# JuliaCrypto/ToyFHE.jl

Measured on AMD Instinct MI355X. Metric: ciphertext-mul/s (BFV ct*ct + relinearize, N=2^14, L=8 RNS), higher is better.
Workload: dtype u64; 1 GPU; BFV N=2^14, L=8 RNS limbs (50-bit primes), extension basis 17 limbs, t=65537, ciphertext-mul + relinearize (RNS-digit keyswitch), bit-exact; batch_per_gpu=1024, global_batch=1024

## Files before the change

toyfhe.jl_amd/csrc/kernels.h:

```cpp
#pragma once
#include <hip/hip_runtime.h>
#include <type_traits>
#include "bfv_core.h"
#include "bfv_fast.h"
#include "lazy_sum.h"
#include "ntt_core.h"

typedef u64 u64x2_t __attribute__((ext_vector_type(2)));

#ifndef TFHE_NTT_WAVES
#define TFHE_NTT_WAVES 2
#endif

__device__ __forceinline__ u32 fresh_tid() {
    u32 t = threadIdx.x;
    asm volatile("" : "+v"(t));
    return t;
}

struct limb_sel_t {
    int n;
    int idx[TFHE_MAX_LIMBS];
};


template <class A, int LOGB, int LOGT, int S0>
__device__ __forceinline__ void fwd_schedule(u64* lds, const u64* gsrc, u64* gdst, const typename A::ctx& C, u32 tid,
                                             u32 pre, int x, u32 sbrev, const lift_t* lift) {
    constexpr int K = pass_k_fwd(LOGB, LOGT, S0);
    constexpr bool LAST = (S0 + K == LOGB);
    ntt_fwd_pass<A, LOGB, LOGT, S0, K, S0 == 0, LAST>(lds, gsrc, gdst, C, tid, pre, x, sbrev, lift);
    if constexpr (!LAST) {
        __syncthreads();
        fwd_schedule<A, LOGB, LOGT, S0 + K>(lds, gsrc, gdst, C, tid, pre, x, sbrev, lift);
    }
}
template <class A, int LOGB, int LOGT, int SEND, bool SCALE = true, class AO = A>
__device__ __forceinline__ void inv_schedule_ptw(u64* lds, const u64* gsrc, u64* gdst, const typename A::ctx& C, u32 tid,
                                                 u32 pre, const u64* addend, const typename A::tw* tw_cur, u64* keep = nullptr) {
    constexpr int K = pass_k_inv(LOGB, LOGT, SEND);
    constexpr int S0 = SEND - K;
    constexpr bool FROM_GLOBAL = (SEND == LOGB), TO_GLOBAL = (S0 == 0);
    typedef pgeom<LOGB, LOGT, S0, K> G;
    u64 raw[G::E];
    typename A::elem v[G::E];
    inv_load_data<LOGB, LOGT, S0, K, FROM_GLOBAL>(raw, lds, gsrc, tid, 0, 0u);
    inv_compute<A, LOGB, LOGT, S0, K, FROM_GLOBAL, SCALE, (TO_GLOBAL || FROM_GLOBAL) ? 0 : K>(v, raw, tw_cur, C, tid, pre);
    if constexpr (!TO_GLOBAL) {
        constexpr int K2 = pass_k_inv(LOGB, LOGT, S0);
        typedef pgeom<LOGB, LOGT, S0 - K2, K2> G2;
        typename A::tw tw_next[G2::SETS * G2::NTW];
        if constexpr (S0 - K2 != 0) inv_load_tw<A, LOGB, LOGT, S0 - K2, K2, false>(tw_next, C, tid, pre);
        inv_store<A, LOGB, LOGT, S0, K, FROM_GLOBAL, SCALE>(v, lds, gdst, C, tid, nullptr);
        __syncthreads();
        inv_schedule_ptw<A, LOGB, LOGT, S0, SCALE, AO>(lds, gsrc, gdst, C, tid, pre, addend, tw_next, keep);
    } else {
        inv_store<AO, LOGB, LOGT, S0, K, FROM_GLOBAL, SCALE>(v, lds, gdst, C, tid, addend, keep);
    }
}

template <class A, int LOGB, int LOGT, int SEND, bool SCALE>
__device__ __forceinline__ void inv_schedule(u64* lds, const u64* gsrc, u64* gdst, const typename A::ctx& C, u32 tid,
                                             u32 pre, int x, u32 sbrev, const u64* addend) {
    constexpr int K = pass_k_inv(LOGB, LOGT, SEND);
    constexpr int S0 = SEND - K;
    ntt_inv_pass<A, LOGB, LOGT, S0, K, SEND == LOGB, S0 == 0, SCALE>(lds, gsrc, gdst, C, tid, pre, x, sbrev, addend);
    if constexpr (S0 != 0) {
        __syncthreads();
        inv_schedule<A, LOGB, LOGT, S0, SCALE>(lds, gsrc, gdst, C, tid, pre, x, sbrev, addend);
    }
}

__device__ __forceinline__ u32 xcd_walk_item(u32 it, u32 b, u32 grid, int x, u32 nitems) {
    const u32 nsb = 1u << x;
    if (x == 0 || (grid % (8u * nsb)) != 0u) {
        const u32 item = it * grid + b;
        return item < nitems ? item : ~0u;
    }
    const u32 xcd = b & 7u, slot = b >> 3, groups = (grid >> 3) >> x;
    const u32 row = it * (8u * groups) + xcd * groups + (slot >> x);
    const u32 item = (row << x) | (slot & (nsb - 1u));
    return item < nitems ? item : ~0u;
}
__device__ __forceinline__ u32 xcd_limb_niter(u32 grid, u32 nitems) {
    if (grid & 7u) return (nitems + grid - 1) / grid;
    const u32 per = (nitems + 7u) >> 3, nslots = grid >> 3;
    return (per + nslots - 1) / nslots;
}
__device__ __forceinline__ u32 xcd_limb_walk(u32 it, u32 wg, u32 grid, u32 nb, u32 nitems) {
    if (grid & 7u) {
        const u32 item = it * grid + wg;
        return item < nitems ? item : ~0u;
    }
    const u32 per = (nitems + 7u) >> 3, nslots = grid >> 3, xcd = wg & 7u, slot = wg >> 3;
    const u32 k = it * nslots + slot, idx = xcd * per + k;
    if (k >= per || idx >= nitems) return ~0u;
    const u32 B = nitems / nb, j = idx / B, b = idx - j * B;
    return b * nb + j;
}
__device__ __forceinline__ u32 dense_mask(u32 limbs, u32 mask) { return (limbs & 1u) ? 0u : mask; }
__device__ __forceinline__ u32 dense_count(u32 nitems, int x, u32 limbs, u32 mask) {
    return mask ? ((((nitems >> x) / limbs) * (u32)__popc(mask)) << x) : nitems;
}
__device__ __forceinline__ u32 dense_item(u32 d, int x, u32 limbs, u32 mask) {
    if (!mask || d == ~0u) return d;
    const u32 nact = (u32)__popc(mask), sb = d & ((1u << x) - 1u), pld = d >> x, g = pld / nact, a = pld % nact;
    u32 m = mask;
    for (u32 i = 0; i < a; i++) m &= m - 1u;
    return ((g * limbs + (u32)__ffs((int)m) - 1u) << x) | sb;
}
template <class A, int LOGB, int LOGT, int IOMODE>
__global__ __launch_bounds__(1 << LOGT, TFHE_NTT_WAVES) void k_ntt_fwd_block(const u64* __restrict__ src, u64* __restrict__ dst,
                                                              const ntt_limb_t* __restrict__ LT, limb_sel_t sel, int x,
                                                              u32 nitems, ntt_io_t io) {
    extern __shared__ __attribute__((aligned(16))) u64 lds[];
    const size_t ntot = (size_t)1 << (LOGB + x);
    const u32 dmask = dense_mask((u32)sel.n, io.limb_mask), dn = dense_count(nitems, x, (u32)sel.n, dmask), niter = (dn + gridDim.x - 1) / gridDim.x;
    bool first = true;
    for (u32 it = 0; it < niter; it++) {
        const u32 item = dense_item(xcd_walk_item(it, blockIdx.x, gridDim.x, x, dn), x, (u32)sel.n, dmask);
        if (item == ~0u) continue;
        const u32 sb = item & ((1u << x) - 1), pl = item >> x;
        u32 srow = pl, drow = pl, j = pl % (u32)sel.n;
        lift_t lf;
        const lift_t* lift = nullptr;
        if constexpr (IOMODE == 1) {
            const u32 per_ct = io.level * io.nw, b = pl / per_ct, rem = pl % per_ct, i = rem / io.nw;
            j = rem % io.nw;
            srow = (b * io.polys + io.polys - 1) * io.level + i;
            const ntt_limb_t& Li = LT[sel.idx[i]];
            const ntt_limb_t& Lj = LT[sel.idx[j]];
            lf.qi = Li.q; lf.half = Li.q >> 1; lf.qj = Lj.q; lf.bj = Lj.br;
            if (io.lift_unsigned) lf.qi = lf.half = ~0ull;
            lift_wide_consts<A>(lf);
            lift = &lf;
        }
        if (io.limb_mask && !((io.limb_mask >> j) & 1u)) continue;
        const typename A::ctx C = A::make(LT[sel.idx[j]]);
        if (!first) __syncthreads();
        first = false;
// ... 1201 lines not shown
        u32 mk0[DCH][2], mk1[DCH][2], md0[DCH][2], md1[DCH][2];
#pragma unroll
        for (int ii = 0; ii < DCH; ii++) {
            const int i = i0 + ii < A.level ? i0 + ii : A.level - 1;
            const u64x2_t a = *(const u64x2_t*)(evk + (((size_t)i * 2 + 0) * Lk + A.w.idx[j]) * n + k);
            const u64x2_t d = *(const u64x2_t*)(evk + (((size_t)i * 2 + 1) * Lk + A.w.idx[j]) * n + k);
#pragma unroll
            for (int v = 0; v < 2; v++) {
                mk0[ii][v] = (u32)a[v] & 0x3ffffffu; mk1[ii][v] = (u32)(a[v] >> 26);
                md0[ii][v] = (u32)d[v] & 0x3ffffffu; md1[ii][v] = (u32)(d[v] >> 26);
            }
        }
        for (u32 b = b_lo; b < b_hi; b++) {
            constexpr bool pairs = EPI;
            u64x2_t *s1p, *s2p;
            if (EPI) {
                s1p = (u64x2_t*)(S + epi_pair(b, j, k, (u32)A.nw, n));
                s2p = s1p + 1;
            } else {
                s1p = (u64x2_t*)(S + (((size_t)b * 2 + 0) * A.nw + j) * n + k);
                s2p = (u64x2_t*)(S + (((size_t)b * 2 + 1) * A.nw + j) * n + k);
            }
            u64x2_t p1 = {0, 0}, p2 = {0, 0};
            if (i0) {
                p1 = *s1p; p2 = *s2p;
                if (pairs) { const u64x2_t a = p1, c = p2; p1.x = a.x; p1.y = c.x; p2.x = a.y; p2.y = c.y; }
            }
            acc52 s1[2] = {{p1[0], 0, 0}, {p1[1], 0, 0}}, s2[2] = {{p2[0], 0, 0}, {p2[1], 0, 0}};
            u64x2_t dv[DCH];
#pragma unroll
            for (int ii = 0; ii < DCH; ii++)
                if (i0 + ii < A.level) dv[ii] = *(const u64x2_t*)(dig + (((size_t)b * A.level + i0 + ii) * A.nw + j) * n + k);
#pragma unroll
            for (int ii = 0; ii < DCH; ii++) {
                if (i0 + ii < A.level) {
#pragma unroll
                    for (int v = 0; v < 2; v++) {
                        const u32 d0 = (u32)dv[ii][v] & 0x3ffffffu, d1 = (u32)(dv[ii][v] >> 26);
                        acc52_mac(s1[v], d0, d1, md0[ii][v], md1[ii][v]);
                        acc52_mac(s2[v], d0, d1, mk0[ii][v], mk1[ii][v]);
                    }
                }
            }
            u64x2_t r1, r2;
#pragma unroll
            for (int v = 0; v < 2; v++) {
                u64 lo, hi;
                acc52_fold(s1[v], lo, hi);
                r1[v] = barrett_reduce128(lo, hi, br);
                acc52_fold(s2[v], lo, hi);
                r2[v] = barrett_reduce128(lo, hi, br);
            }
            if constexpr (EPI) {
                if (i0 + DCH >= A.level && j < (u32)K.epi_level) {
                    const u64x2_t x = *(const u64x2_t*)(K.epi_x + (((size_t)b * 2) * K.epi_level + j) * n + k);
#pragma unroll
                    for (int v = 0; v < 2; v++) {
                        r1[v] = addmod(shoup_full(r1[v], A.pinv[j], br.q), x[v], br.q);
                        r2[v] = shoup_full(r2[v], A.pinv[j], br.q);
                    }
                }
            }
            if (pairs) {
                u64x2_t a, c;
                a.x = r1[0]; a.y = r2[0]; c.x = r1[1]; c.y = r2[1];
                *s1p = a;
                *s2p = c;
            } else {
                *s1p = r1;
                *s2p = r2;
            }
        }
    }
}

template <class A, int LOGB, int LOGT, bool PRELIFT = false>
__device__ __forceinline__ void fused_fwd_to_regs(u64* lds, const u64* grow, const typename A::ctx& C, bool& first,
                                                  typename A::elem* v, const lift_t* lift = nullptr) {
    constexpr int K1 = pass_k_fwd(LOGB, LOGT, 0), K2 = pass_k_fwd(LOGB, LOGT, K1), K3 = LOGB - K1 - K2;
    constexpr int E = 1 << (LOGB - LOGT);
    const u32 tid = fresh_tid();
    {
        u64 raw[E];
        fwd_load_data<LOGB, LOGT, 0, K1, true, false>(raw, lds, grow, tid);
        if (!first) __syncthreads();
        first = false;
        if constexpr (PRELIFT) {
#pragma unroll
            for (int i = 0; i < E; i++) pin_vgpr(raw[i]);
            TFHE_SCHED_FENCE();
            fwd_compute<A, LOGB, LOGT, 0, K1, false, false, 0>(v, raw, nullptr, C, tid, 1u);
        } else {
            fwd_compute<A, LOGB, LOGT, 0, K1, true, false, 0>(v, raw, nullptr, C, tid, 1u, lift);
        }
        fwd_store<A, LOGB, LOGT, 0, K1, false>(v, lds, nullptr, C, tid, 0, 0u);
    }
    __syncthreads();
    ntt_fwd_pass<A, LOGB, LOGT, K1, K2, false, false>(lds, nullptr, nullptr, C, tid, 1u, 0, 0u);
    __syncthreads();
    {
        u64 r3[E];
        fwd_load_data<LOGB, LOGT, K1 + K2, K3, false, true>(r3, lds, nullptr, tid);
        fwd_compute<A, LOGB, LOGT, K1 + K2, K3, false, true, 0>(v, r3, nullptr, C, tid, 1u);
    }
}
template <class A, int LOGB, int LOGT, bool SCALE = true, class AO = A>
__device__ __forceinline__ void fused_inv_from_regs(u64* lds, typename A::elem* v, u64* gdst, const typename A::ctx& C, const u64* addend,
                                                    u64* keep = nullptr, u32 pre = 1u) {
    constexpr int KI1 = pass_k_inv(LOGB, LOGT, LOGB);
    constexpr int E = 1 << (LOGB - LOGT);
    const u32 tid = fresh_tid();
    __syncthreads();
    constexpr int S1 = LOGB - KI1, K2 = pass_k_inv(LOGB, LOGT, S1);
    typedef pgeom<LOGB, LOGT, S1 - K2, K2> G2;
    typename A::tw tw_next[G2::SETS * G2::NTW];
    {
#pragma unroll
        for (int e = 0; e < E; e++) v[e] = fp_reduce(v[e], C.p, C.pinv);
        inv_compute<A, LOGB, LOGT, S1, KI1, true, SCALE, 0, -1, no_hook, true>(v, nullptr, nullptr, C, tid, pre);
        if constexpr (S1 - K2 != 0) inv_load_tw<A, LOGB, LOGT, S1 - K2, K2, false>(tw_next, C, tid, pre);
        inv_store<A, LOGB, LOGT, S1, KI1, true, SCALE>(v, lds, nullptr, C, tid);
    }
    __syncthreads();
    inv_schedule_ptw<A, LOGB, LOGT, S1, SCALE, AO>(lds, nullptr, gdst, C, tid, pre, addend, tw_next, keep);
}

template <class A, int LOGB, int LOGT>
__global__ __launch_bounds__(1 << LOGT) void k_ntt_inv_quad2(const u64* __restrict__ src, u64* __restrict__ dst,
                                                              const ntt_limb_t* __restrict__ LT, limb_sel_t sel, u32 nitems, u32 limb_mask) {
    extern __shared__ __attribute__((aligned(16))) u64 lds[];
    constexpr int x = 2;
    constexpr int K1 = pass_k_inv(LOGB, LOGT, LOGB), S1 = LOGB - K1;
    typedef pgeom<LOGB, LOGT, S1, K1> G1;
    constexpr int E = G1::E;
    constexpr int K2 = pass_k_inv(LOGB, LOGT, S1), KL = S1 - K2;
    static_assert(KL >= 1 && pass_k_inv(LOGB, LOGT, KL) == KL, "three-pass schedule expected");
    typedef pgeom<LOGB, LOGT, 0, KL> GL;
    static_assert(GL::SETS == 1 && GL::LO == LOGT, "last pass: element r of a thread is word tid + (r << LOGT)");
    static_assert(G1::SETS << (LOGT + K1) == 1 << LOGB, "first pass: register position e <-> point tid + (e << LOGT)");
    const size_t ntot = (size_t)1 << (LOGB + x);
    const u32 dmask = dense_mask((u32)sel.n, limb_mask), dn = dense_count(nitems, 1, (u32)sel.n, dmask), niter = (dn + gridDim.x - 1) / gridDim.x;
    bool first = true;
    for (u32 it = 0; it < niter; it++) {
        const u32 item = dense_item(xcd_walk_item(it, blockIdx.x, gridDim.x, x - 1, dn), 1, (u32)sel.n, dmask);
        if (item == ~0u) continue;
        const u32 ph = item & 1u, pl = item >> 1, j = pl % (u32)sel.n;
        if (limb_mask && !((limb_mask >> j) & 1u)) continue;
        const ntt_limb_t& L = LT[sel.idx[j]];
        typename A::ctx C = A::make(L);
        C.Winvb = L.i2_winvb;
        const u64* s = src + pl * ntot;
        u64* d = dst + pl * ntot + 2u * ph;
        typename A::elem w[2][E];
        {
            const u32 tid = fresh_tid();
            typedef __attribute__((address_space(1))) const double* gptr_t;
            const gptr_t t0 = (gptr_t)L.i2_t0;
            double ta = ph ? t0[(1u << LOGT) + tid] : 1.0;
            double tb = t0[(ph ? (2u << LOGT) : 0u) + tid];
            const ftw_t ga{ph ? L.i2_g[1] : 1.0}, gb{ph ? L.i2_g[2] : L.i2_g[0]}, iinv{L.i2_iinv};
            const double sgn = ph ? -1.0 : 1.0;
            pin_vgpr(ta);
            pin_vgpr(tb);
            if (!first) __syncthreads();
            dma_stream_load<LOGB, LOGT, 4, 2>(lds, s, tid, [&](int e, const u64* q) {
                const int idx = (e % G1::SETS) * G1::R + (int)brev_bits((u32)(e / G1::SETS), K1);
                const double a0 = fp_from_u64(q[0]), a1 = fp_from_u64(q[1]), a2 = fp_from_u64(q[2]), a3 = fp_from_u64(q[3]);
                asm volatile("" : "+v"(ta), "+v"(tb) : "v"(a0));
                const double slo = fp_fma(sgn, a1 + a3, a0 + a2);
                const double t = fp_mulmod_c(a1 - a3, iinv, C.p, C.pinv);
                const double shi = fp_fma(sgn, t, a0 - a2);
                w[0][idx] = fp_mulmod_c(slo, ftw_t{ta}, C.p, C.pinv);
                w[1][idx] = fp_mulmod_c(shi, ftw_t{tb}, C.p, C.pinv);
                ta = fp_mulmod_c(ta, ga, C.p, C.pinv);
                tb = fp_mulmod_c(tb, gb, C.p, C.pinv);
            });
            first = false;
            TFHE_SCHED_FENCE();
        }
        u64 held[E];
#pragma unroll
        for (int half = 0; half < 2; half++) {
            const u32 tid = fresh_tid();
            TFHE_SCHED_FENCE();
            __syncthreads();
            {
                typename A::elem* v = w[half];
#pragma unroll
                for (int e = 0; e < E; e++) v[e] = fp_reduce(v[e], C.p, C.pinv);
                inv_compute<A, LOGB, LOGT, S1, K1, true, true, 0, -1, no_hook, true>(v, nullptr, nullptr, C, tid, 1u);
                inv_store<A, LOGB, LOGT, S1, K1, true, true>(v, lds, nullptr, C, tid);
            }
            __syncthreads();
            ntt_inv_pass<A, LOGB, LOGT, KL, K2, false, false, true>(lds, nullptr, nullptr, C, tid, 1u, 0, 0u);
            __syncthreads();
            {
                u64 r3[E];
                typename A::elem v[E];
                inv_load_data<LOGB, LOGT, 0, KL, false>(r3, lds, nullptr, tid, 0, 0u);
                inv_compute<A, LOGB, LOGT, 0, KL, false, true, 0>(v, r3, nullptr, C, tid, 1u);
                if (half == 0) {
#pragma unroll
                    for (int r = 0; r < E; r++) held[r] = A::out_inv_scaled(v[r], C);
                } else {
#pragma unroll
                    for (int r = 0; r < E; r++) {
                        u64x2_t ww;
// ... 26 lines not shown
        d[pair ? pos * 2 : pos] = b;
    }
}
template <int LOGB, int LOGT>
constexpr size_t fused_lds_bytes() {
    return (size_t)lds_words<LOGB, LOGT>() * 8;
}
template <class A, int LOGB, int LOGT, bool PRELIFT = false, int SPMODE = 0>
__global__ __launch_bounds__(1 << LOGT) void k_ks_fused(const u64* __restrict__ evd, const u64* __restrict__ ct,
                                                         u64* __restrict__ out, const ntt_limb_t* __restrict__ LT,
                                                         ks_arg_t KA, int Lk, u32 nitems, const u64* __restrict__ tsp = nullptr,
                                                         const u64* __restrict__ zero_row = nullptr) {
    extern __shared__ __attribute__((aligned(16))) u64 lds[];
    constexpr int K1 = pass_k_fwd(LOGB, LOGT, 0), K2 = pass_k_fwd(LOGB, LOGT, K1), K3 = LOGB - K1 - K2;
    static_assert(K3 >= 1 && pass_k_fwd(LOGB, LOGT, K1 + K2) == K3, "three-pass forward schedule expected");
    constexpr int KI1 = pass_k_inv(LOGB, LOGT, LOGB);
    static_assert(KI1 == K3, "forward last pass and inverse first pass must share the register map");
    typedef pgeom<LOGB, LOGT, 0, K1> G1;
    typedef pgeom<LOGB, LOGT, K1 + K2, K3> G3;
    constexpr int E = G3::E;
    const u32 level = (u32)KA.level, polys = (u32)KA.polys, nw = (u32)KA.nw;
    const u32 add_s = polys == 3 ? 2u : 1u;
    bool first = true;
    const u32 niter = (nitems + gridDim.x - 1) / gridDim.x;
    for (u32 it = 0; it < niter; it++) {
        const u32 nper = SPMODE == 1 ? 1u : (SPMODE >= 2 ? level : nw);
        const u32 item = it * gridDim.x + blockIdx.x;
        if (item >= nitems) break;
        const u32 b = item / nper, j = SPMODE == 1 ? level : item % nper;
        const ntt_limb_t& Lj = LT[KA.w.idx[j]];
        typename A::ctx C = A::make(Lj);
        lift_t lf;
        lf.qj = Lj.q;
        lf.bj = Lj.br;
        typename A::elem acc[2][E];
#pragma unroll
        for (int e = 0; e < E; e++) acc[0][e] = acc[1][e] = 0;
        for (u32 i = 0; i < level; i++) {
            const u32 tid = fresh_tid();
            lf.qi = LT[KA.w.idx[i]].q;
            lf.half = lf.qi >> 1;
            const u64* grow = ct + ((size_t)((b * polys + polys - 1) * level + i) << LOGB);
            typename A::elem v[E];
            fused_fwd_to_regs<A, LOGB, LOGT, PRELIFT>(lds, grow, C, first, v, &lf);
            const u64x2_t* e_pair = (const u64x2_t*)(evd + ((((size_t)i * nw + j) << LOGB) << 1));
#pragma unroll
            for (int u = 0; u < G3::SETS; u++) {
                u32 c0, hi, base;
                G3::template coords<true>(tid, u, c0, hi, base);
#pragma unroll
                for (int r = 0; r < G3::R; r++) {
                    const u32 nat = (brev_bits((u32)r, K3) << (LOGB - K3)) + c0;
                    const int e = u * G3::R + r;
                    const u64x2_t kw = e_pair[nat];
                    const typename A::tw k1{A::from_lds(kw.y)}, k0{A::from_lds(kw.x)};
                    const double y = A::pre_product(v[e], C);
                    acc[0][e] += fp_mulmod_c(y, k1, C.p, C.pinv);
                    acc[1][e] += fp_mulmod_c(y, k0, C.p, C.pinv);
                }
            }
            if ((i & 7u) == 7u && i + 1 < level) {
#pragma unroll
                for (int e = 0; e < E; e++) {
                    acc[0][e] = fp_reduce(acc[0][e], C.p, C.pinv);
                    acc[1][e] = fp_reduce(acc[1][e], C.p, C.pinv);
                }
            }
        }
#pragma unroll
        for (int sidx = 0; sidx < 2; sidx++) {
            if constexpr (SPMODE >= 2) {
                C.md_pinv = (double)KA.pinv[j].w;
                C.md_c = (u32)sidx < add_s ? ct + ((size_t)((b * polys + sidx) * level + j) << LOGB) : zero_row;
                C.md_g = KA.rot_g;
                u64* gdst = out + ((size_t)((b * 2 + sidx) * level + j) << LOGB);
                typedef typename std::conditional<SPMODE == 3, ArithFpMDR, ArithFpMD>::type AOUT;
                fused_inv_from_regs<A, LOGB, LOGT, false, AOUT>(lds, acc[sidx], gdst, C, tsp + ((size_t)(b * 2 + sidx) << LOGB));
            } else if constexpr (SPMODE == 1) {
                u64* gdst = out + ((size_t)(b * 2 + sidx) << LOGB);
                fused_inv_from_regs<A, LOGB, LOGT, false>(lds, acc[sidx], gdst, C, nullptr);
            } else {
                const u64* addend = (!KA.special && (u32)sidx < add_s) ? ct + ((size_t)((b * polys + sidx) * level + j) << LOGB) : nullptr;
                u64* gdst = out + ((size_t)((b * 2 + sidx) * nw + j) << LOGB);
                fused_inv_from_regs<A, LOGB, LOGT, false>(lds, acc[sidx], gdst, C, addend);
            }
        }
    }
}

template <class A, int LOGB, int LOGT, int X>
__global__ __launch_bounds__(1 << LOGT) void k_ks_fused_sub(const u64* __restrict__ evd, const u64* __restrict__ ct,
                                                             u64* __restrict__ T, const ntt_limb_t* __restrict__ LT,
                                                             ks_arg_t KA, int Lk, u32 nitems) {
    extern __shared__ __attribute__((aligned(16))) u64 lds[];
    constexpr int K1 = pass_k_fwd(LOGB, LOGT, 0), K2 = pass_k_fwd(LOGB, LOGT, K1), K3 = LOGB - K1 - K2;
    static_assert(K3 >= 1 && pass_k_fwd(LOGB, LOGT, K1 + K2) == K3, "three-pass forward schedule expected");
    constexpr int KI1 = pass_k_inv(LOGB, LOGT, LOGB), S1 = LOGB - KI1;
    static_assert(KI1 == K3, "forward last pass and inverse first pass must share the register map");
    typedef pgeom<LOGB, LOGT, K1 + K2, K3> G3;
    constexpr int E = G3::E;
    const u32 level = (u32)KA.level, polys = (u32)KA.polys, nw = (u32)KA.nw;
    const u32 niter = (nitems + gridDim.x - 1) / gridDim.x;
    bool first = true;
    for (u32 it = 0; it < niter; it++) {
        const u32 item = xcd_walk_item(it, blockIdx.x, gridDim.x, X, nitems);
        if (item == ~0u) continue;
        const u32 sb = item & ((1u << X) - 1u), pl = item >> X, b = pl / nw, j = pl % nw, pre = (1u << X) + sb;
        const ntt_limb_t& Lj = LT[KA.w.idx[j]];
        const typename A::ctx C = A::make(Lj);
        lift_t lf;
        lf.qj = Lj.q;
        lf.bj = Lj.br;
        const typename A::tw w1 = A::ld_fwd(C, 1u), w2 = A::ld_fwd(C, 2u + (sb >> 1));
        const double sgn_h = (sb >> (X - 1)) ? -1.0 : 1.0, sgn_q = (sb & 1u) ? -1.0 : 1.0;
        typename A::elem acc[2][E];
#pragma unroll
        for (int e = 0; e < E; e++) acc[0][e] = acc[1][e] = 0;
        for (u32 i = 0; i < level; i++) {
            const u32 tid = fresh_tid();
            lf.qi = LT[KA.w.idx[i]].q;
            lf.half = lf.qi >> 1;
            const u64* grow = ct + ((size_t)((b * polys + polys - 1) * level + i) << (LOGB + X));
            typename A::elem v[E];
            {
                u64 op[E];
                constexpr int PC = 4 * X, PE = E / PC;
                if constexpr (X == 2) {
                    if (!first) __syncthreads();
                    dma_stream_load<LOGB, LOGT, 1 << X, 2>(lds, grow, tid, [&](int e, const u64* q) {
                        double xin[1 << X];
#pragma unroll
                        for (int m = 0; m < (1 << X); m++) xin[m] = A::from_global_lift(q[m], C, lf, true);
                        double z;
                        if constexpr (X == 1) {
                            z = fp_fma(sgn_h, fp_mulmod_c(xin[1], w1, C.p, C.pinv), xin[0]);
                        } else {
                            const double ya = fp_fma(sgn_h, fp_mulmod_c(xin[2], w1, C.p, C.pinv), xin[0]);
                            const double yb = fp_fma(sgn_h, fp_mulmod_c(xin[3], w1, C.p, C.pinv), xin[1]);
                            z = fp_fma(sgn_q, fp_mulmod_c(yb, w2, C.p, C.pinv), ya);
                        }
                        op[e] = A::to_lds(A::top_reduce(z, C));
                    });
                } else
#pragma unroll
                for (int h = 0; h < PC; h++) {
                    u64 q[1 << X][PE];
                    u32 tp = tid;
                    if (h > 0) order_after(tp, op[h * PE - 1]);
#pragma unroll
                    for (int r = 0; r < PE; r++) {
                        const u32 k = tp + ((u32)(h * PE + r) << LOGT);
#pragma unroll
                        for (int m = 0; m < (1 << X); m++) {
                            q[m][r] = grow[k + ((u32)m << LOGB)];
                        }
                    }
                    TFHE_SCHED_FENCE();
#pragma unroll
                    for (int r = 0; r < PE; r++) {
                        double xin[1 << X];
#pragma unroll
                        for (int m = 0; m < (1 << X); m++) xin[m] = A::from_global_lift(q[m][r], C, lf, true);
                        double z;
                        if constexpr (X == 1) {
                            z = fp_fma(sgn_h, fp_mulmod_c(xin[1], w1, C.p, C.pinv), xin[0]);
                        } else {
                            const double ya = fp_fma(sgn_h, fp_mulmod_c(xin[2], w1, C.p, C.pinv), xin[0]);
// ... 591 lines not shown
                for (int r = 0; r < R; r++) p[r] = neg[r] ? negmod(p[r], LP.q) : p[r];
            }
            constexpr u32 JB = X == 1 ? 4 : 2;
            const bool addc = s < add_s;
            for (u32 j0 = team; j0 < level; j0 += teams * JB) {
                u64 v[JB][R], cv[JB][R];
#pragma unroll
                for (u32 t = 0; t < JB; t++) {
                    const u32 j = j0 + t * teams < level ? j0 + t * teams : j0;
                    const u64* tj = T + ((size_t)pr * A.nw + j) * n;
                    const u64* c = ct + (((size_t)b * A.polys + (addc ? s : 0u)) * level + j) * n;
#pragma unroll
                    for (int r = 0; r < R; r++) {
                        v[t][r] = tj[k + (u32)r * stride];
                        cv[t][r] = addc ? c[k + (u32)r * stride] : 0;
                    }
                }
#pragma unroll
                for (u32 t = 0; t < JB; t++) {
                    const u32 j = j0 + t * teams;
                    if (j < level) {
                        const ntt_limb_t& L = LT[A.w.idx[j]];
                        const u64 q = L.q;
                        u64* o = out + ((size_t)pr * level + j) * n;
                        ntt_inv_top_regs<X>(v[t], L);
#pragma unroll
                        for (int r = 0; r < R; r++) {
                            u64 x = neg[r] ? negmod(v[t][r], q) : v[t][r];
                            if (A.special) x = shoup_full(submod(x, barrett_reduce128(p[r], 0, L.br), q), ra.qlinv[j], q);
                            if (addc) x = addmod(x, neg[r] ? negmod(cv[t][r], q) : cv[t][r], q);
                            o[m[r]] = x;
                        }
                    }
                }
            }
        }
    }
}

#define BFV_BS 128
__global__ __launch_bounds__(BFV_BS) void k_bfv_expand(const u64* __restrict__ src, u64* __restrict__ dst,
                                                        const bfv_tab_t* __restrict__ Bt, u32 n, u32 gx) {
    extern __shared__ __attribute__((aligned(16))) u64 lds[];
    const bfv_tab_t& B = *Bt;
    const u32 k = (blockIdx.x % gx) * BFV_BS + threadIdx.x;
    const size_t p = blockIdx.x / gx;
    if (k >= n) return;
    bfv_expand_coeff(B, src + p * B.ns * n + k, n, dst + p * B.nb * n + k, n, lds + threadIdx.x, BFV_BS);
}
__global__ __launch_bounds__(BFV_BS) void k_bfv_contract(const u64* __restrict__ src, u64* __restrict__ dst,
                                                          const bfv_tab_t* __restrict__ Bt, u32 n, u32 gx) {
    extern __shared__ __attribute__((aligned(16))) u64 lds[];
    const bfv_tab_t& B = *Bt;
    const u32 k = (blockIdx.x % gx) * BFV_BS + threadIdx.x;
    const size_t p = blockIdx.x / gx;
    if (k >= n) return;
    u64* xi = lds + threadIdx.x;
    u64* zb = xi + (size_t)B.nb * BFV_BS;
    u64* rb = zb + (size_t)B.nb * BFV_BS;
    bfv_contract_coeff(B, src + p * B.nb * n + k, n, dst + p * B.ns * n + k, n, xi, zb, rb, BFV_BS);
}

template <int NS, int NP, bool NARROW>
__global__ __launch_bounds__(256) void k_bfv_expand_fast(const u64* __restrict__ src, u64* __restrict__ dst,
                                                          const bfv_fast_tab_t* __restrict__ Bt, u32 n, u32 gx, int copy_shared) {
    const u32 k = (blockIdx.x % gx) * 256 + threadIdx.x;
    const size_t p = blockIdx.x / gx;
    if (k >= n) return;
    if constexpr (NARROW) {
        __shared__ u64 col[(NS > NP ? NS : NP) * 256];
        bfv_expand_narrow<NS, NP>(*Bt, src + p * NS * n + k, n, dst + p * (NS + NP) * n + k, n, col + threadIdx.x, 256, copy_shared != 0);
    }
    else bfv_expand_fast<NS, NP, false>(*Bt, src + p * NS * n + k, n, dst + p * (NS + NP) * n + k, n, copy_shared != 0);
}
template <int NS, int NP, bool NARROW, bool LIFT3 = false, bool TD = false, bool FOLDED = false>
__global__ __launch_bounds__(256) void k_bfv_contract_fast(const u64* __restrict__ src, u64* __restrict__ dst,
                                                            const bfv_fast_tab_t* __restrict__ Bt, u32 n, u32 gx) {
    const u32 k = (blockIdx.x % gx) * 256 + threadIdx.x;
    const u32 b = blockIdx.x / gx;
    const size_t p = b;
    if (k >= n) return;
    if constexpr (NARROW) {
        __shared__ u64 col[(NS > NP ? NS : NP) * 256];
        bfv_contract_narrow<NS, NP, TD, FOLDED>(*Bt, src + p * (NS + NP) * n + k, n, dst + p * NS * n + k, n, col + threadIdx.x, 256, LIFT3 && b % 3u == 2u);
    } else {
        bfv_contract_fast<NS, NP, false>(*Bt, src + p * (NS + NP) * n + k, n, dst + p * NS * n + k, n);
    }
}

#include "ks_group_core.h"
```

toyfhe.jl_amd/csrc/ntt_core.h:

```cpp
#pragma once
#include "fp64arith.h"
#include "modarith.h"

#if defined(__HIP_DEVICE_COMPILE__)
#define TFHE_SCHED_FENCE() asm volatile("" ::: "memory")
#else
#define TFHE_SCHED_FENCE() ((void)0)
#endif

struct alignas(16) twd_t {
    u64 w, wp;
};
TFHE_HD tw_t as_tw(const twd_t& t) { return tw_t{t.w, t.wp}; }
TFHE_HD tw_t ld_tw(const twd_t* tab, u32 i) {
#if defined(__HIP_DEVICE_COMPILE__)
    typedef __attribute__((address_space(1))) const twd_t* gptr_t;
    const gptr_t g = (gptr_t)tab;
    return tw_t{g[i].w, g[i].wp};
#else
    return tw_t{tab[i].w, tab[i].wp};
#endif
}

template <int LOGB, int LOGT>
// ... 240 lines not shown
    for (int S = logb; S > 0;) {
        if (S == send) return b;
        const int K = pass_k_inv(logb, logt, S), S0 = S - K;
        const double out = fps_inv_growth(b, K);
        const bool red = S0 > 0 && fps_inv_growth(out, pass_k_inv(logb, logt, S0)) > TFHE_FPS_LIMIT;
        b = red ? 0.502 : out;
        S = S0;
    }
    return b;
}
struct ArithFpS : ArithFp {
    static constexpr bool fwd_sweep_before(int, int) { return false; }
    static constexpr double fp_a = TFHE_FPS_A, fp_lim = TFHE_FPS_LIMIT;
    template <int LOGB, int LOGT, int S0> static constexpr bool inv_lds_reduce() { return fps_inv_reduce(LOGB, LOGT, S0); }
    template <int LOGB, int LOGT, int SEND> static constexpr double inv_entry() { return fps_inv_entry(LOGB, LOGT, SEND); }
    static TFHE_HD elem pre_product(elem v, const ctx&) { return v; }
    static TFHE_HD elem top_reduce(elem v, const ctx&) { return v; }
};

struct ntt_io_t {
    u32 mode;
    u32 gsz;
    u32 src_gstride;
    u32 dst_gstride;
    u32 level, nw, polys;
    u32 add_rows;
    u32 add_gstride;
    const u64* addend;
    u32 limb_mask;
    u32 lift_unsigned;
};

template <int LOGB, int LOGT, int S0, int K>
struct pgeom {
    static constexpr int T = 1 << LOGT, E = 1 << (LOGB - LOGT), R = 1 << K, SETS = E >> K, LO = LOGB - S0 - K;
    static constexpr int NTW = R - 1;
    static_assert(K >= 1 && (E >> K) >= 1, "pass wider than the per-thread register block");
    template <bool BREV>
    static TFHE_HD void coords(u32 tid, int u, u32& c0, u32& hi, u32& base) {
        c0 = (u32)u * T + tid;
        const u32 c = BREV ? brev_bits(c0, LOGB - K) : c0;
        const u32 lo = c & ((1u << LO) - 1);
        hi = (!BREV && SETS == 1 && LO >= LOGT) ? 0u : c >> LO;
        base = (hi << (LOGB - S0)) + lo;
    }
};

template <class A, int LOGB, int LOGT, int S0, int K, bool LAST, int D0 = 0, int D1 = K>
TFHE_HD void fwd_load_tw(typename A::tw* tw, const typename A::ctx& C, u32 tid, u32 pre) {
    typedef pgeom<LOGB, LOGT, S0, K> G;
#pragma unroll
    for (int u = 0; u < G::SETS; u++) {
        u32 c0, hi, base;
        G::template coords<LAST>(tid, u, c0, hi, base);
#pragma unroll
        for (int d = D0; d < D1; d++)
#pragma unroll
            for (int g = 0; g < (1 << d); g++)
                tw[u * G::NTW + (1 << d) - 1 + g] = (LAST && A::has_b(C))
                                                        ? A::ld_fwd_b(C, (pre << (S0 + d)) + (c0 << d) + (u32)g)
                                                        : A::ld_fwd(C, (pre << (S0 + d)) + (hi << d) + (u32)g);
    }
}
TFHE_HD u64 xchg_rd(const u64* lds, u32 i) { return lds[i]; }
TFHE_HD void xchg_wr(u64* lds, u32 i, u64 v) { lds[i] = v; }
template <int LOGB, int LOGT, int S0, int K, bool FIRST, bool LAST, int USEL = -1>
TFHE_HD void fwd_load_data(u64* raw, const u64* lds, const u64* gsrc, u32 tid, const lift_t* lift = nullptr) {
    typedef pgeom<LOGB, LOGT, S0, K> G;
#pragma unroll
    for (int u = 0; u < G::SETS; u++) {
        if (USEL >= 0 && u != USEL) continue;
        u32 c0, hi, base;
        G::template coords<LAST>(tid, u, c0, hi, base);
        const u32 pb = FIRST ? 0u : lds_phi<LOGB, LOGT>(base);
#pragma unroll
        for (int r = 0; r < G::R; r++) {
            const u32 j = base + ((u32)r << G::LO);
            raw[u * G::R + r] = FIRST ? gsrc[j] : xchg_rd(lds, pb + lds_phi_c<LOGB, LOGT>((u32)r << G::LO));
        }
    }
    TFHE_SCHED_FENCE();
    (void)lift;
}
template <class A, int LOGB, int LOGT, int S0, int K, bool FIRST, bool LAST, int PF, int USEL = -1, class HOOK = no_hook>
TFHE_HD void fwd_compute(typename A::elem* v, const u64* raw, const typename A::tw* twp, const typename A::ctx& C, u32 tid,
                         u32 pre, const lift_t* lift = nullptr, const HOOK& hook = HOOK(), u64* lds_early = nullptr) {
    typedef pgeom<LOGB, LOGT, S0, K> G;
    const bool use_b = LAST && A::has_b(C);
    if (FIRST && lift) {
#pragma unroll
        for (int i = 0; i < G::E; i++) v[i] = A::from_global_lift(raw[i], C, *lift, true);
        TFHE_SCHED_FENCE();
    }
#pragma unroll
    for (int u = 0; u < G::SETS; u++) {
        if (USEL >= 0 && u != USEL) continue;
        u32 c0, hi, base;
        G::template coords<LAST>(tid, u, c0, hi, base);
        typename A::elem* vv = v + u * G::R;
#pragma unroll
        for (int r = 0; r < G::R; r++) {
            if (FIRST && lift) continue;
            vv[r] = FIRST ? A::from_global_plain(raw[u * G::R + r], C) : A::from_lds(raw[u * G::R + r]);
        }
#pragma unroll
        for (int d = 0; d < K; d++) {
            const int half = 1 << (K - 1 - d);
            if (A::fwd_sweep_before(LOGB, S0 + d)) {
#pragma unroll
                for (int r = 0; r < G::R; r++) A::range_fwd(vv[r], C);
            }
#pragma unroll
            for (int g = 0; g < (1 << d); g++) {
                const typename A::tw w = d < PF ? twp[u * G::NTW + (1 << d) - 1 + g]
                                         : (LAST && use_b) ? A::ld_fwd_b(C, (pre << (S0 + d)) + (c0 << d) + (u32)g)
                                                           : A::ld_fwd(C, (pre << (S0 + d)) + (hi << d) + (u32)g);
#pragma unroll
                for (int i = 0; i < half; i++) {
                    const int r0 = (g << (K - d)) + i;
                    A::bf_fwd(vv[r0], vv[r0 + half], w, C);
                    if (!LAST && lds_early && d == K - 1) {
                        const u32 pb = lds_phi<LOGB, LOGT>(base);
                        xchg_wr(lds_early, pb + lds_phi_c<LOGB, LOGT>((u32)r0 << G::LO), A::to_lds(vv[r0]));
                        xchg_wr(lds_early, pb + lds_phi_c<LOGB, LOGT>((u32)(r0 + 1) << G::LO), A::to_lds(vv[r0 + 1]));
                    }
                }
                hook(((u * K + d) * (G::R / 2)) + g * half, ((u * K + d) * (G::R / 2)) + (g + 1) * half, G::SETS * K * (G::R / 2));
            }
        }
    }
}
template <class A, int LOGB, int LOGT, int S0, int K, bool LAST, int USEL = -1>
TFHE_HD void fwd_store(typename A::elem* v, u64* lds, u64* gdst, const typename A::ctx& C, u32 tid, int x, u32 sb_rev) {
    typedef pgeom<LOGB, LOGT, S0, K> G;
    static_assert(!LAST || G::LO == 0, "LAST pass must end at stage LOGB-1");
#pragma unroll
    for (int u = 0; u < G::SETS; u++) {
        if (USEL >= 0 && u != USEL) continue;
        u32 c0, hi, base;
        G::template coords<LAST>(tid, u, c0, hi, base);
        const u32 pb = LAST ? 0u : lds_phi<LOGB, LOGT>(base);
#pragma unroll
        for (int r = 0; r < G::R; r++) {
            typename A::elem e = v[u * G::R + r];
            if (LAST) {
                const u32 nat = (brev_bits((u32)r, K) << (LOGB - K)) + c0;
                gdst[((u64)nat << x) + sb_rev] = A::out_fwd(e, C);
            } else {
                xchg_wr(lds, pb + lds_phi_c<LOGB, LOGT>((u32)r << G::LO), A::to_lds(e));
            }
        }
    }
}
template <class A, int LOGB, int LOGT, int S0, int K, bool FIRST, bool LAST, bool ES = false>
TFHE_HD void ntt_fwd_pass(u64* lds, const u64* gsrc, u64* gdst, const typename A::ctx& C, u32 tid, u32 pre, int x,
                          u32 sb_rev, const lift_t* lift = nullptr) {
    typedef pgeom<LOGB, LOGT, S0, K> G;
    u64 raw[G::E];
    typename A::elem v[G::E];
    fwd_load_data<LOGB, LOGT, S0, K, FIRST, LAST>(raw, lds, gsrc, tid);
    if constexpr (!LAST && ES) {
        fwd_compute<A, LOGB, LOGT, S0, K, FIRST, LAST, 0>(v, raw, nullptr, C, tid, pre, FIRST ? lift : nullptr, no_hook(), lds);
    } else {
        fwd_compute<A, LOGB, LOGT, S0, K, FIRST, LAST, 0>(v, raw, nullptr, C, tid, pre, FIRST ? lift : nullptr);
        fwd_store<A, LOGB, LOGT, S0, K, LAST>(v, lds, gdst, C, tid, x, sb_rev);
    }
// ... 31 lines not shown
            }
        }
    }
    TFHE_SCHED_FENCE();
}
struct inv_plan_t {
    u32 mask[8];
};
template <int K>
constexpr inv_plan_t make_inv_plan(double a = TFHE_FP_A, double lim = TFHE_FP_LIMIT, double b0 = 0.502) {
    inv_plan_t P{};
    double b[1 << K] = {};
    for (int i = 0; i < (1 << K); i++) b[i] = b0;
    for (int st = 0; st < K; st++) {
        const int d = K - 1 - st, half = 1 << st;
        for (int g = 0; g < (1 << d); g++)
            for (int i = 0; i < half; i++) {
                const int r0 = (g << (K - d)) + i, r1 = r0 + half;
                while (b[r0] + b[r1] > lim) {
                    const int m = b[r0] >= b[r1] ? r0 : r1;
                    b[m] = 0.502;
                    P.mask[st] |= 1u << m;
                }
                const double sm = b[r0] + b[r1];
                b[r0] = sm;
                b[r1] = 0.5 + 1.5 * a * sm + 0.002;
            }
    }
    return P;
}

template <class A, int LOGB, int LOGT, int S0, int K, bool FROM_GLOBAL, bool SCALE, int PF, int USEL = -1, class HOOK = no_hook,
          bool PRE = false>
TFHE_HD void inv_compute(typename A::elem* v, const u64* raw, const typename A::tw* twp, const typename A::ctx& C, u32 tid,
                         u32 pre, const HOOK& hook = HOOK(), u64* lds_early = nullptr) {
    typedef pgeom<LOGB, LOGT, S0, K> G;
    const bool use_b = FROM_GLOBAL && A::has_b(C);
#pragma unroll
    for (int u = 0; u < G::SETS; u++) {
        if (USEL >= 0 && u != USEL) continue;
        u32 c0, hi, base;
        G::template coords<FROM_GLOBAL>(tid, u, c0, hi, base);
        typename A::elem* vv = v + u * G::R;
#pragma unroll
        for (int r = 0; r < G::R; r++)
            if (!PRE) vv[r] = FROM_GLOBAL ? A::from_global(raw[u * G::R + r], C) : A::from_lds(raw[u * G::R + r]);
#pragma unroll
        for (int d = K - 1; d >= 0; d--) {
            const int half = 1 << (K - 1 - d);
            {
                constexpr inv_plan_t PLAN = make_inv_plan<K>(A::fp_a, A::fp_lim, A::template inv_entry<LOGB, LOGT, S0 + K>());
#pragma unroll
                for (int r = 0; r < G::R; r++)
                    if ((PLAN.mask[K - 1 - d] >> r) & 1u) A::range_inv(vv[r], C);
            }
#pragma unroll
            for (int g = 0; g < (1 << d); g++) {
                if (SCALE && S0 == 0 && d == 0) {
#pragma unroll
                    for (int i = 0; i < half; i++) A::bf_inv_scaled(vv[i], vv[i + half], C);
                } else {
                    const typename A::tw w = d >= K - PF ? twp[u * G::NTW + (1 << d) - 1 + g]
                                             : (FROM_GLOBAL && use_b) ? A::ld_inv_b(C, (pre << (S0 + d)) + (c0 << d) + (u32)g)
                                                                      : A::ld_inv(C, (pre << (S0 + d)) + (hi << d) + (u32)g);
#pragma unroll
                    for (int i = 0; i < half; i++) {
                        const int r0 = (g << (K - d)) + i;
                        A::bf_inv(vv[r0], vv[r0 + half], w, C);
                        if (S0 != 0 && lds_early && d == 0) {
                            const u32 pb = lds_phi<LOGB, LOGT>(base);
                            typename A::elem e0 = vv[r0], e1 = vv[r0 + half];
                            if (A::template inv_lds_reduce<LOGB, LOGT, S0>()) { A::range_inv(e0, C); A::range_inv(e1, C); }
                            xchg_wr(lds_early, pb + lds_phi_c<LOGB, LOGT>((u32)r0 << G::LO), A::to_lds(e0));
                            xchg_wr(lds_early, pb + lds_phi_c<LOGB, LOGT>((u32)(r0 + half) << G::LO), A::to_lds(e1));
                        }
                    }
                }
                hook(((u * K + (K - 1 - d)) * (G::R / 2)) + g * half, ((u * K + (K - 1 - d)) * (G::R / 2)) + (g + 1) * half,
                     G::SETS * K * (G::R / 2));
            }
        }
    }
}
template <class A, int LOGB, int LOGT, int S0, int K, bool FROM_GLOBAL, bool SCALE, int USEL = -1>
TFHE_HD void inv_store(typename A::elem* v, u64* lds, u64* gdst, const typename A::ctx& C, u32 tid,
                       const u64* addend = nullptr, u64* keep = nullptr) {
    typedef pgeom<LOGB, LOGT, S0, K> G;
    constexpr bool TO_GLOBAL = (S0 == 0);
    if constexpr (TO_GLOBAL) {
        if (keep) {
#pragma unroll
            for (int i = 0; i < G::E; i++) keep[i] = SCALE ? A::out_inv_scaled(v[i], C) : A::out_inv_lazy(v[i], C);
            return;
        }
        u32 pos[G::SETS];
#pragma unroll
        for (int u = 0; u < G::SETS; u++) {
            u32 c0, hi;
            G::template coords<FROM_GLOBAL>(tid, u, c0, hi, pos[u]);
        }
        if (addend) {
            constexpr bool MD = A::moddown;
            constexpr int NB = G::E >= 8 ? (MD && G::E >= 16 ? 8 : 4) : 1, BS = G::E / NB;
            u64 add[2][BS], add2[2][MD ? BS : 1];
            auto request = [&](int q) {
#pragma unroll
                for (int k = 0; k < BS; k++) {
                    const int e = q * BS + k, u = e / G::R, r = e % G::R;
                    if (USEL >= 0 && u != USEL) continue;
                    add[q & 1][k] = addend[pos[u] + ((u32)r << G::LO)];
                    if constexpr (MD) add2[q & 1][k] = C.md_c[pos[u] + ((u32)r << G::LO)];
                }
                TFHE_SCHED_FENCE();
            };
            request(0);
#pragma unroll
            for (int q = 0; q < NB; q++) {
                if (q + 1 < NB) request(q + 1);
                u64 o[BS];
#pragma unroll
                for (int k = 0; k < BS; k++) {
                    if constexpr (MD) {
                        if constexpr (A::rot) {
                            const int e = q * BS + k, u = e / G::R, r = e % G::R;
                            const u32 t = ((pos[u] + ((u32)r << G::LO)) * C.md_g) & ((2u << LOGB) - 1u);
                            o[k] = A::out_moddown_rot(v[q * BS + k], add[q & 1][k], add2[q & 1][k], (t >> LOGB) != 0, C);
                        } else {
                            o[k] = A::out_moddown(v[q * BS + k], add[q & 1][k], add2[q & 1][k], C);
                        }
                    } else o[k] = SCALE ? A::out_inv_scaled(v[q * BS + k], C) : A::out_inv_lazy(v[q * BS + k], C);
                }
                TFHE_SCHED_FENCE();
#pragma unroll
                for (int k = 0; k < BS; k++) {
                    const int e = q * BS + k, u = e / G::R, r = e % G::R;
                    if (USEL >= 0 && u != USEL) continue;
                    if constexpr (MD) {
                        if constexpr (A::rot) gdst[((pos[u] + ((u32)r << G::LO)) * C.md_g) & ((1u << LOGB) - 1u)] = o[k];
                        else gdst[pos[u] + ((u32)r << G::LO)] = o[k];
                    } else gdst[pos[u] + ((u32)r << G::LO)] = addmod(o[k], add[q & 1][k], C.q);
                }
                TFHE_SCHED_FENCE();
            }
        } else {
            u64 o[G::E];
#pragma unroll
            for (int i = 0; i < G::E; i++) o[i] = SCALE ? A::out_inv_scaled(v[i], C) : A::out_inv_lazy(v[i], C);
            TFHE_SCHED_FENCE();
#pragma unroll
            for (int e = 0; e < G::E; e++) {
                const int u = e / G::R, r = e % G::R;
                if (USEL >= 0 && u != USEL) continue;
                gdst[pos[u] + ((u32)r << G::LO)] = o[e];
            }
        }
    } else {
#pragma unroll
        for (int u = 0; u < G::SETS; u++) {
            if (USEL >= 0 && u != USEL) continue;
            u32 c0, hi, base;
            G::template coords<FROM_GLOBAL>(tid, u, c0, hi, base);
#pragma unroll
            for (int r = 0; r < G::R; r++) {
                typename A::elem e = v[u * G::R + r];
                if (A::template inv_lds_reduce<LOGB, LOGT, S0>()) A::range_inv(e, C);
                xchg_wr(lds, lds_phi<LOGB, LOGT>(base) + lds_phi_c<LOGB, LOGT>((u32)r << G::LO), A::to_lds(e));
            }
        }
    }
}
template <class A, int LOGB, int LOGT, int S0, int K, bool FROM_GLOBAL, bool TO_GLOBAL, bool SCALE, bool ES = false>
TFHE_HD void ntt_inv_pass(u64* lds, const u64* gsrc, u64* gdst, const typename A::ctx& C, u32 tid, u32 pre, int x,
                          u32 sb_rev, const u64* addend = nullptr) {
    typedef pgeom<LOGB, LOGT, S0, K> G;
    static_assert(TO_GLOBAL == (S0 == 0), "TO_GLOBAL pass is the one ending at stage 0");
    u64 raw[G::E];
    typename A::elem v[G::E];
    inv_load_data<LOGB, LOGT, S0, K, FROM_GLOBAL>(raw, lds, gsrc, tid, x, sb_rev);
    if constexpr (ES && !TO_GLOBAL) {
        inv_compute<A, LOGB, LOGT, S0, K, FROM_GLOBAL, SCALE, 0>(v, raw, nullptr, C, tid, pre, no_hook(), lds);
    } else {
        inv_compute<A, LOGB, LOGT, S0, K, FROM_GLOBAL, SCALE, 0>(v, raw, nullptr, C, tid, pre);
        inv_store<A, LOGB, LOGT, S0, K, FROM_GLOBAL, SCALE>(v, lds, gdst, C, tid, TO_GLOBAL ? addend : nullptr);
    }
}

template <int X>
TFHE_HD void ntt_fwd_top(const u64* src, u64* dst, const twd_t* W, u64 q, u64 col, u64 stride) {
    constexpr int R = 1 << X;
    u64 v[R];
#pragma unroll
    for (int r = 0; r < R; r++) v[r] = src[col + (u64)r * stride];
#pragma unroll
    for (int d = 0; d < X; d++) {
// ... 69 lines not shown
```

Baseline: 64070 ciphertext-mul/s.

## Use paired-word layout for prelifted rows to enable 128-bit loads

```diff
diff --git a/toyfhe.jl_amd/csrc/kernels.h b/toyfhe.jl_amd/csrc/kernels.h
--- a/toyfhe.jl_amd/csrc/kernels.h
+++ b/toyfhe.jl_amd/csrc/kernels.h
@@ -35,7 +35,7 @@
         fwd_schedule<A, LOGB, LOGT, S0 + K>(lds, gsrc, gdst, C, tid, pre, x, sbrev, lift);
     }
 }
-template <class A, int LOGB, int LOGT, int SEND, bool SCALE = true, class AO = A>
+template <class A, int LOGB, int LOGT, int SEND, bool SCALE = true, class AO = A, int ROWS = ROWS_NATURAL>
 __device__ __forceinline__ void inv_schedule_ptw(u64* lds, const u64* gsrc, u64* gdst, const typename A::ctx& C, u32 tid,
                                                  u32 pre, const u64* addend, const typename A::tw* tw_cur, u64* keep = nullptr) {
     constexpr int K = pass_k_inv(LOGB, LOGT, SEND);
@@ -53,9 +53,9 @@
         if constexpr (S0 - K2 != 0) inv_load_tw<A, LOGB, LOGT, S0 - K2, K2, false>(tw_next, C, tid, pre);
         inv_store<A, LOGB, LOGT, S0, K, FROM_GLOBAL, SCALE>(v, lds, gdst, C, tid, nullptr);
         __syncthreads();
-        inv_schedule_ptw<A, LOGB, LOGT, S0, SCALE, AO>(lds, gsrc, gdst, C, tid, pre, addend, tw_next, keep);
+        inv_schedule_ptw<A, LOGB, LOGT, S0, SCALE, AO, ROWS>(lds, gsrc, gdst, C, tid, pre, addend, tw_next, keep);
     } else {
-        inv_store<AO, LOGB, LOGT, S0, K, FROM_GLOBAL, SCALE>(v, lds, gdst, C, tid, addend, keep);
+        inv_store<AO, LOGB, LOGT, S0, K, FROM_GLOBAL, SCALE, -1, ROWS>(v, lds, gdst, C, tid, addend, keep);
     }
 }
 
@@ -1423,7 +1423,8 @@
     const u32 tid = fresh_tid();
     {
         u64 raw[E];
-        fwd_load_data<LOGB, LOGT, 0, K1, true, false>(raw, lds, grow, tid);
+        if constexpr (PRELIFT) fwd_load_data_pair<LOGB, LOGT, K1>(raw, grow, tid);
+        else fwd_load_data<LOGB, LOGT, 0, K1, true, false>(raw, lds, grow, tid);
         if (!first) __syncthreads();
         first = false;
         if constexpr (PRELIFT) {
@@ -1445,7 +1446,7 @@
         fwd_compute<A, LOGB, LOGT, K1 + K2, K3, false, true, 0>(v, r3, nullptr, C, tid, 1u);
     }
 }
-template <class A, int LOGB, int LOGT, bool SCALE = true, class AO = A>
+template <class A, int LOGB, int LOGT, bool SCALE = true, class AO = A, int ROWS = ROWS_NATURAL>
 __device__ __forceinline__ void fused_inv_from_regs(u64* lds, typename A::elem* v, u64* gdst, const typename A::ctx& C, const u64* addend,
                                                     u64* keep = nullptr, u32 pre = 1u) {
     constexpr int KI1 = pass_k_inv(LOGB, LOGT, LOGB);
@@ -1463,7 +1464,7 @@
         inv_store<A, LOGB, LOGT, S1, KI1, true, SCALE>(v, lds, nullptr, C, tid);
     }
     __syncthreads();
-    inv_schedule_ptw<A, LOGB, LOGT, S1, SCALE, AO>(lds, nullptr, gdst, C, tid, pre, addend, tw_next, keep);
+    inv_schedule_ptw<A, LOGB, LOGT, S1, SCALE, AO, ROWS>(lds, nullptr, gdst, C, tid, pre, addend, tw_next, keep);
 }
 
 template <class A, int LOGB, int LOGT>
@@ -1656,7 +1657,7 @@
             } else {
                 const u64* addend = (!KA.special && (u32)sidx < add_s) ? ct + ((size_t)((b * polys + sidx) * level + j) << LOGB) : nullptr;
                 u64* gdst = out + ((size_t)((b * 2 + sidx) * nw + j) << LOGB);
-                fused_inv_from_regs<A, LOGB, LOGT, false>(lds, acc[sidx], gdst, C, addend);
+                fused_inv_from_regs<A, LOGB, LOGT, false, A, PRELIFT ? ROWS_PAIR_ADDEND : ROWS_NATURAL>(lds, acc[sidx], gdst, C, addend);
             }
         }
     }
@@ -2414,7 +2415,8 @@
     if (k >= n) return;
     if constexpr (NARROW) {
         __shared__ u64 col[(NS > NP ? NS : NP) * 256];
-        bfv_contract_narrow<NS, NP, TD, FOLDED>(*Bt, src + p * (NS + NP) * n + k, n, dst + p * NS * n + k, n, col + threadIdx.x, 256, LIFT3 && b % 3u == 2u);
+        const u32 ks = LIFT3 ? pair_coeff_n(k, n) : k;
+        bfv_contract_narrow<NS, NP, TD, FOLDED>(*Bt, src + p * (NS + NP) * n + ks, n, dst + p * NS * n + k, n, col + threadIdx.x, 256, LIFT3 && b % 3u == 2u);
     } else {
         bfv_contract_fast<NS, NP, false>(*Bt, src + p * (NS + NP) * n + k, n, dst + p * NS * n + k, n);
     }
diff --git a/toyfhe.jl_amd/csrc/ntt_core.h b/toyfhe.jl_amd/csrc/ntt_core.h
--- a/toyfhe.jl_amd/csrc/ntt_core.h
+++ b/toyfhe.jl_amd/csrc/ntt_core.h
@@ -346,6 +346,41 @@
     TFHE_SCHED_FENCE();
     (void)lift;
 }
+struct alignas(16) u64pair_t {
+    u64 x, y;
+};
+template <int LOGB, int LOGT>
+TFHE_HD u32 pair_pos(u32 k) {
+    static_assert(LOGB - LOGT >= 1, "a thread owns at least two words");
+    const u32 tid = k & ((1u << LOGT) - 1u), e = k >> LOGT;
+    return ((e >> 1) << (LOGT + 1)) + 2u * tid + (e & 1u);
+}
+template <int LOGB, int LOGT>
+TFHE_HD u32 pair_coeff(u32 p) {
+    static_assert(LOGB - LOGT >= 1, "a thread owns at least two words");
+    const u32 w = p & ((2u << LOGT) - 1u), e = ((p >> (LOGT + 1)) << 1) | (w & 1u);
+    return (w >> 1) + (e << LOGT);
+}
+TFHE_HD u32 pair_coeff_n(u32 p, u32 n) {
+    const u32 logt = (u32)logt_for(__builtin_ctz(n));
+    const u32 w = p & ((2u << logt) - 1u), e = ((p >> (logt + 1)) << 1) | (w & 1u);
+    return (w >> 1) + (e << logt);
+}
+template <int LOGB, int LOGT, int K>
+TFHE_HD void fwd_load_data_pair(u64* raw, const u64* gsrc, u32 tid) {
+    typedef pgeom<LOGB, LOGT, 0, K> G;
+    static_assert(G::SETS == 1 && G::LO == LOGT, "first pass: element r of a thread is word tid + (r << LOGT)");
+    const u64pair_t* const g = (const u64pair_t*)gsrc + tid;
+#pragma unroll
+    for (int h = 0; h < G::E / 2; h++) {
+        const u64pair_t w = g[(u32)h << LOGT];
+        raw[2 * h] = w.x;
+        raw[2 * h + 1] = w.y;
+    }
+    TFHE_SCHED_FENCE();
+}
+enum { ROWS_NATURAL = 0, ROWS_PAIR_ADDEND = 1 };
+
 template <class A, int LOGB, int LOGT, int S0, int K, bool FIRST, bool LAST, int PF, int USEL = -1, class HOOK = no_hook>
 TFHE_HD void fwd_compute(typename A::elem* v, const u64* raw, const typename A::tw* twp, const typename A::ctx& C, u32 tid,
                          u32 pre, const lift_t* lift = nullptr, const HOOK& hook = HOOK(), u64* lds_early = nullptr) {
@@ -543,11 +578,13 @@
         }
     }
 }
-template <class A, int LOGB, int LOGT, int S0, int K, bool FROM_GLOBAL, bool SCALE, int USEL = -1>
+template <class A, int LOGB, int LOGT, int S0, int K, bool FROM_GLOBAL, bool SCALE, int USEL = -1, int ROWS = ROWS_NATURAL>
 TFHE_HD void inv_store(typename A::elem* v, u64* lds, u64* gdst, const typename A::ctx& C, u32 tid,
                        const u64* addend = nullptr, u64* keep = nullptr) {
     typedef pgeom<LOGB, LOGT, S0, K> G;
     constexpr bool TO_GLOBAL = (S0 == 0);
+    static_assert(ROWS == ROWS_NATURAL || (TO_GLOBAL && G::SETS == 1 && G::LO == LOGT && USEL < 0 && !A::moddown && G::E >= 8),
+                  "pair order: last pass, element r of a thread is word tid + (r << LOGT)");
     if constexpr (TO_GLOBAL) {
         if (keep) {
 #pragma unroll
@@ -569,8 +606,15 @@
                 for (int k = 0; k < BS; k++) {
                     const int e = q * BS + k, u = e / G::R, r = e % G::R;
                     if (USEL >= 0 && u != USEL) continue;
-                    add[q & 1][k] = addend[pos[u] + ((u32)r << G::LO)];
-                    if constexpr (MD) add2[q & 1][k] = C.md_c[pos[u] + ((u32)r << G::LO)];
+                    if constexpr ((ROWS & ROWS_PAIR_ADDEND) != 0) {
+                        if (k & 1) continue;
+                        const u64pair_t w = ((const u64pair_t*)addend)[tid + ((u32)(e >> 1) << LOGT)];
+                        add[q & 1][k] = w.x;
+                        add[q & 1][k + 1] = w.y;
+                    } else {
+                        add[q & 1][k] = addend[pos[u] + ((u32)r << G::LO)];
+                        if constexpr (MD) add2[q & 1][k] = C.md_c[pos[u] + ((u32)r << G::LO)];
+                    }
                 }
                 TFHE_SCHED_FENCE();
             };
```

Result: no change. 64420 ciphertext-mul/s (median of 5 runs) (+0.5%).
